# ethz-asl/laser_slam

Measured on AMD Instinct MI355X. Metric: scans_per_sec, higher is better.
Workload: dtype f32

## Files before the change

laser_slam_amd/csrc/lsgpu_icp.hip:

```cpp
#include <cstring>
#include <cmath>
#include <cstdio>
#include <cstdlib>
#include <string>
#include <vector>
#include <chrono>
#include <system_error>
#include <thread>
#include <utility>

#include <dlfcn.h>

#include <hip/hip_runtime.h>
#include <rccl/rccl.h>

#include "../../include/lsgpu_icp.h"
#include "lsgpu_grid.hip.h"
#include "lsgpu_tuning.h"
#include "lsgpu_policy.h"
#include "lsgpu_knn.hip.h"
#include "lsgpu_knn_k.hip.h"
#include "lsgpu_snf.hip.h"
#include "lsgpu_max_density.hip.h"
#include "lsgpu_cone.hip.h"
// ... 1683 lines not shown
    const bool fresh = h->ssn_bounds_ws.cap == 0;
    HIPC(h->ssn_bounds_ws.reserve(8 + 6 * kSsnBoundsBlocks));
    if (fresh) HIPC(hipMemsetAsync(h->ssn_bounds_ws.p, 0, 8 * sizeof(uint32_t), h->stream));
    hipLaunchKernelGGL(k_ssn_bounds_root, dim3(std::min(nblk(n), kSsnBoundsBlocks)), dim3(256), 0, h->stream, src, (int)n, h->ssn_bounds_ws.p,
                       h->ssn_bb.p, h->ssn_seg_a.p);
  }
  SsnSeg* cur = h->ssn_seg_a.p;
  SsnSeg* nxt = h->ssn_seg_b.p;
  const uint32_t* idx = nullptr;
  const int* root_axis = nullptr;
  int glevels = 0;
  const int root_auto = n >= 200ll * 8192 ? 8192 : n >= 200ll * 4096 ? 4096 : 2048;
  const int root_max = tuning().ssn_root ? tuning().ssn_root : root_auto;
  int root_levels = 0;
  while ((8 << root_levels) < root_max) ++root_levels;
  {
    int64_t c = n;
    while (glevels < levels && !(c <= root_max && levels - glevels <= root_levels)) { c -= c / 2; ++glevels; }
  }
  const bool select_levels = !force_sort_levels && !tuning().ssn_sort_levels && glevels > 0;
  const uint32_t* root_sig = nullptr;
  if (select_levels) {
    if (h->gs_plan_n != n || h->gs_plan_levels != glevels) {
      std::vector<uint32_t> sizes{(uint32_t)n}, next;
      h->gs_lvl_first.clear(); h->gs_lvl_blocks.clear();
      uint32_t rows = 0, segs = 0;
      for (int L = 0; L < glevels; ++L) {
        uint32_t fb = 0;
        next.clear();
        for (uint32_t c : sizes) {
          fb += (c + kGsTile - 1u) / kGsTile;
          next.push_back(c - c / 2u); next.push_back(c / 2u);
        }
        h->gs_lvl_first.push_back(rows); h->gs_lvl_blocks.push_back(fb);
        rows += fb; segs += (uint32_t)sizes.size();
        sizes.swap(next);
      }
      HIPC(h->gs_tab.reserve(rows)); HIPC(h->gs_sblk.reserve(segs));
      if (glevels <= kGsPlanLevels && ((size_t)1 << (glevels - 1)) <= kGsPlanSegs) {
        GsPlanArgs pa{};
        for (int L = 0; L < glevels; ++L) pa.first[L] = h->gs_lvl_first[L];
        hipLaunchKernelGGL(k_gs_plan, dim3(glevels), dim3(1024), 0, h->stream, (uint32_t)n, pa, h->gs_tab.p, h->gs_sblk.p);
        HIPC(hipGetLastError());
      } else {
        std::vector<GsBlock> tab;
        std::vector<GsSegBlocks> sblk;
        std::vector<std::pair<uint32_t, uint32_t>> segsz{{0u, (uint32_t)n}};
        for (int L = 0; L < glevels; ++L) {
          uint32_t fb = 0;
          std::vector<std::pair<uint32_t, uint32_t>> nx;
          for (uint32_t sidx = 0; sidx < segsz.size(); ++sidx) {
            const uint32_t st = segsz[sidx].first, c = segsz[sidx].second;
            const uint32_t nb = (c + kGsTile - 1u) / kGsTile;
            sblk.push_back(GsSegBlocks{fb, nb, st, c});
            for (uint32_t k = 0; k < nb; ++k)
              tab.push_back(GsBlock{st + k * kGsTile, std::min(kGsTile, c - k * kGsTile), sidx, st, c, fb, nb, 0u});
            fb += nb;
            const uint32_t left = c - c / 2u;
            nx.push_back({st, left}); nx.push_back({st + left, c - left});
          }
          segsz.swap(nx);
        }
        HIPC(hipMemcpyAsync(h->gs_tab.p, tab.data(), tab.size() * sizeof(GsBlock), hipMemcpyHostToDevice, h->stream));
        HIPC(hipMemcpyAsync(h->gs_sblk.p, sblk.data(), sblk.size() * sizeof(GsSegBlocks), hipMemcpyHostToDevice, h->stream));
        HIPC(hipStreamSynchronize(h->stream));
      }
      h->gs_plan_n = n; h->gs_plan_levels = glevels;
    }
    const size_t nseg_g = (size_t)1 << glevels;
    int cap = 1;
    for (uint32_t v : h->gs_lvl_blocks) cap = std::max(cap, (int)v);
    for (auto& bf : h->gs_e) HIPC(bf.reserve(n));
    for (auto& bf : h->gs_k) HIPC(bf.reserve(n));
    HIPC(h->gs_hist.reserve(4 * 256 * (nseg_g + 1))); HIPC(h->gs_median.reserve(nseg_g)); HIPC(h->gs_cand_n.reserve(2 * nseg_g + 2));
    const size_t cand_room = std::max<size_t>(nseg_g / 2, 1) * kGsCandRoom;
    HIPC(h->gs_cand.reserve(cand_room)); HIPC(h->gs_cand_blk.reserve(cand_room));
    HIPC(h->gs_cl.reserve((size_t)2 * cap)); HIPC(h->gs_err.reserve(8)); HIPC(h->gs_rng.reserve(2 * nseg_g + 2));
    HIPC(h->ssn_axis_a.reserve(nseg_g)); HIPC(h->ssn_axis_b.reserve(nseg_g));
    if (!h->h_gs_err) HIPC(hipHostMalloc((void**)&h->h_gs_err, 64, hipHostMallocDefault));
    uint32_t* cand_n[2] = {h->gs_cand_n.p, h->gs_cand_n.p + nseg_g + 1};
    uint32_t* sig_cur = reinterpret_cast<uint32_t*>(h->ssn_axis_a.p);
    uint32_t* sig_nxt = reinterpret_cast<uint32_t*>(h->ssn_axis_b.p);
    GsSet in, out;
    in.e = h->gs_e[0].p; out.e = h->gs_e[1].p;
    for (int d = 0; d < 3; ++d) { in.k[d] = h->gs_k[d].p; out.k[d] = h->gs_k[3 + d].p; }
    uint2* rng_cur = h->gs_rng.p;
    uint2* rng_nxt = h->gs_rng.p + nseg_g + 1;
    uint32_t* gh1[2] = {h->gs_hist.p, h->gs_hist.p + 256 * (nseg_g + 1)};
    uint32_t* gh2[2] = {h->gs_hist.p + 2 * 256 * (nseg_g + 1), h->gs_hist.p + 3 * 256 * (nseg_g + 1)};
    hipLaunchKernelGGL(k_gs_init, dim3(nblk(n)), dim3(256), 0, h->stream, src, (int)n, in, out.e, (const SsnSeg*)cur, (const uint32_t*)h->ssn_bb.p, rng_cur,
                       gh1[0], gh2[0], cand_n[0], sig_cur, h->gs_err.p);
    for (int L = 0; L < glevels; ++L) {
      const int ns = 1 << L, nb = (int)h->gs_lvl_blocks[L], par = L & 1;
      const GsBlock* tab = h->gs_tab.p + h->gs_lvl_first[L];
      const GsSegBlocks* sblk = h->gs_sblk.p + (ns - 1);
      hipLaunchKernelGGL(k_gs_hist<1>, dim3(nb), dim3(256), 0, h->stream, tab, cur, (const uint2*)rng_cur, in, gh1[par], gh2[par], h->gs_err.p);
      hipLaunchKernelGGL(k_gs_hist<2>, dim3(nb), dim3(256), 0, h->stream, tab, cur, (const uint2*)rng_cur, in, gh1[par], gh2[par], h->gs_err.p);
      const uint32_t lvl_cap = (uint32_t)std::min<size_t>(cand_room / (size_t)ns, (size_t)1 << 22);
      hipLaunchKernelGGL(k_gs_collect, dim3(nb), dim3(256), 0, h->stream, tab, cur, (const uint2*)rng_cur, (const uint32_t*)sig_cur, in,
                         (const uint32_t*)gh1[par], (const uint32_t*)gh2[par], cand_n[par], h->gs_cand.p, h->gs_cand_blk.p, lvl_cap, h->gs_cl.p);
      hipLaunchKernelGGL(k_gs_select, dim3(ns), dim3(L < 3 ? 1024 : 256), 0, h->stream, sblk, src, cur, (const uint32_t*)sig_cur, gh1[par], gh2[par],
                         gh1[par ^ 1], gh2[par ^ 1], cand_n[par], (const GsMedian*)h->gs_cand.p, (const uint32_t*)h->gs_cand_blk.p, lvl_cap, h->gs_cl.p,
                         h->gs_cl.p + cap, h->gs_median.p, nxt, sig_nxt, cand_n[par ^ 1], rng_nxt, h->gs_err.p);
      hipLaunchKernelGGL(k_gs_part, dim3(nb), dim3(kGsPartThreads), 0, h->stream, tab, cur, (const uint32_t*)sig_cur, in, out,
                         (const GsMedian*)h->gs_median.p, (const uint32_t*)(h->gs_cl.p + cap), (const SsnSeg*)nxt, rng_nxt, h->gs_err.p);
      std::swap(in, out);
      std::swap(cur, nxt);
      std::swap(sig_cur, sig_nxt);
      std::swap(rng_cur, rng_nxt);
    }
    idx = in.e;
    root_sig = sig_cur;
    HIPC(hipGetLastError());
  } else if (glevels > 0) {
    const size_t nseg_g = (size_t)1 << glevels;
    const int cap = (int)(n / kSegTile + (int64_t)(nseg_g / 2) + 2);
    HIPC(h->lane.scratch->vals_alt.reserve(n));
    HIPC(h->ssn_axis_a.reserve(nseg_g)); HIPC(h->ssn_axis_b.reserve(nseg_g)); HIPC(h->ssn_seg_fb.reserve(nseg_g));
    HIPC(h->ssn_blocktab.reserve((size_t)cap)); HIPC(h->lane.scratch->sort_hist.reserve((size_t)256 * cap + 256 + 4));
    uint32_t* keyA = reinterpret_cast<uint32_t*>(h->lane.scratch->keys.p);
    uint32_t* keyB = keyA + n;
    uint32_t* valA = h->lane.scratch->vals.p;
    uint32_t* valB = h->lane.scratch->vals_alt.p;
    uint32_t* bh = h->lane.scratch->sort_hist.p;
    uint32_t* dtot = bh + (size_t)256 * cap;
    uint32_t* nblocks_dev = dtot + 256;
    int* ax_cur = h->ssn_axis_a.p;
    int* ax_nxt = h->ssn_axis_b.p;
    HIPC(hipMemsetAsync(ax_cur, 0xFF, sizeof(int), h->stream));
    for (int L = 0; L < glevels; ++L) {
      const int ns = 1 << L;
      const int grid = (int)std::min<int64_t>(cap, n / kSegTile + ns + 1);
      hipLaunchKernelGGL(k_ssn_plan, dim3(1), dim3(256), 0, h->stream, cur, ns, knn, ax_cur, h->ssn_seg_fb.p,
                         h->ssn_blocktab.p, nblocks_dev);
      hipLaunchKernelGGL(k_ssn_keys32, dim3(nblk(n)), dim3(256), 0, h->stream, src, (int)n, valA, h->ssn_seg_of.p, cur,
                         h->ssn_seg_fb.p, L == 0 ? 1 : 0, keyA);
      for (int pass = 0; pass < 4; ++pass) {
        const uint32_t* kin = (pass & 1) ? keyB : keyA; const uint32_t* vin = (pass & 1) ? valB : valA;
        uint32_t* kout = (pass & 1) ? keyA : keyB; uint32_t* vout = (pass & 1) ? valA : valB;
        hipLaunchKernelGGL(k_seg_hist<kSegItems>, dim3(grid), dim3(256), 0, h->stream, kin, h->ssn_blocktab.p, nblocks_dev, 8 * pass, bh, cap);
        hipLaunchKernelGGL(k_seg_scan, dim3(256), dim3(256), 0, h->stream, bh, cap, nblocks_dev, dtot);
        hipLaunchKernelGGL((k_seg_scatter<kSegItems>), dim3(grid), dim3(256), 0, h->stream, kin, vin, kout, vout,
                           h->ssn_blocktab.p, nblocks_dev, 8 * pass, bh, dtot, cap);
      }
      idx = valA;
      hipLaunchKernelGGL(k_ssn_split, dim3(nblk(ns)), dim3(256), 0, h->stream, src, idx, cur, ns, knn, nxt, (const int*)ax_cur, ax_nxt);
      hipLaunchKernelGGL(k_ssn_assign, dim3(nblk(n)), dim3(256), 0, h->stream, (int)n, cur, knn, h->ssn_seg_of.p, L == 0 ? 1 : 0);
      std::swap(cur, nxt);
      std::swap(ax_cur, ax_nxt);
    }
    root_axis = ax_cur;
    HIPC(hipGetLastError());
  }
  if (glevels < levels) {
    if (glevels == 0) {
      hipLaunchKernelGGL(k_ssn_keys, dim3(nblk(n)), dim3(256), 0, h->stream, src, (int)n, (const uint32_t*)nullptr,
                         (const uint32_t*)nullptr, cur, knn, h->lane.scratch->keys.p, h->lane.scratch->vals.p);
      idx = h->lane.scratch->vals.p;
    }
    uint32_t* idx_rw = const_cast<uint32_t*>(idx);
    if (root_max == 8192)
      hipLaunchKernelGGL(k_ssn_tree<8192>, dim3(1 << glevels), dim3(1024), 0, h->stream, src, idx_rw, cur, knn, levels - glevels, h->ssn_seg_of.p, nxt, root_axis, root_sig);
    else if (root_max == 4096)
      hipLaunchKernelGGL(k_ssn_tree<4096>, dim3(1 << glevels), dim3(512), 0, h->stream, src, idx_rw, cur, knn, levels - glevels, h->ssn_seg_of.p, nxt, root_axis, root_sig);
    else
      hipLaunchKernelGGL(k_ssn_tree<2048>, dim3(1 << glevels), dim3(256), 0, h->stream, src, idx_rw, cur, knn, levels - glevels, h->ssn_seg_of.p, nxt, root_axis, root_sig);
    std::swap(cur, nxt);
  }
  if (levels == 0) {
    hipLaunchKernelGGL(k_ssn_keys, dim3(nblk(n)), dim3(256), 0, h->stream, src, (int)n, (const uint32_t*)nullptr,
                       (const uint32_t*)nullptr, cur, knn, h->lane.scratch->keys.p, h->lane.scratch->vals.p);
    HIPC(hipMemsetAsync(h->ssn_seg_of.p, 0, (size_t)n * 4, h->stream));
    idx = h->lane.scratch->vals.p;
  }
  hipLaunchKernelGGL(k_ssn_boxes, dim3((int)((nseg + 127) / 128)), dim3(128), 0, h->stream, src, idx, cur, (int)nseg,
                     h->ssn_box_normal.p, h->ssn_box_pts.p);
  HIPC(hipGetLastError());
  int rc = scan_u32(h, h->ssn_box_pts.p, h->ssn_box_base.p, nseg);
  if (rc) return rc;
  rc = ahead->ready(first_draw + (size_t)n);
  if (rc) return rc;
  hipLaunchKernelGGL(k_ssn_select, dim3(nblk(n)), dim3(256), 0, h->stream, (int)n, idx, h->ssn_seg_of.p, cur,
                     h->ssn_box_pts.p, h->ssn_box_base.p, h->ssn_draws.p + first_draw, ratio, h->ssn_keep.p);
  rc = scan_u32(h, h->ssn_keep.p, h->ssn_out_pos.p, (size_t)n, false,  true);
  if (rc == LSGPU_OK) {
    hipLaunchKernelGGL(k_ssn_emit, dim3(nblk(n)), dim3(256), 0, h->stream, src, (int)n,
                       h->ssn_box_normal.p, h->ssn_keep.p, h->ssn_out_pos.p, out_xyz1, out_nrm);
  }
  uint32_t n_draws = 0, kept = 0;
  if (rc == LSGPU_OK)
    rc = scan_totals(h, h->ssn_box_pts.p, h->ssn_box_base.p, nseg, h->ssn_keep.p, h->ssn_out_pos.p, (size_t)n, &n_draws, &kept,
                     select_levels ? h->gs_err.p : nullptr, h->h_gs_err, 8 * sizeof(uint32_t),  true);
  if (rc) return rc;
  if (select_levels && *h->h_gs_err) {
    if (getenv("LSGPU_GS_DEBUG")) fprintf(stderr, "lsgpu: sort-free levels gave up (n %lld): code %u seg %u a %u b %u | part %u seg %u dst %u\n", (long long)n,
                                          h->h_gs_err[1], h->h_gs_err[2], h->h_gs_err[3], h->h_gs_err[4], h->h_gs_err[5], h->h_gs_err[6], h->h_gs_err[7]);
    ++h->ssn_sort_fallbacks;
    return ssn_device(h, src, n, knn, ratio, seed, out_xyz1, out_nrm, n_out, ahead, true);
  }
  ahead->used = first_draw + (size_t)n_draws;
  HIPC(hipGetLastError());
  *n_out = kept;
  return LSGPU_OK;
}

static int random_sampling_device(lsgpu_icp* h, const float4* src, int64_t n, float prob, int64_t seed,
                                  float4* out_xyz1, int64_t* n_out, DrawAhead* ahead = nullptr, bool defer_wait = false) {
  *n_out = 0;
  HIPC(h->ssn_keep.reserve(n));
  HIPC(h->ssn_out_pos.reserve(n));
  DrawAhead own;
  int rc = LSGPU_OK;
  if (!ahead) {
    rc = own.begin(h, seed, (size_t)n);
    if (rc) return rc;
    ahead = &own;
  }
  const size_t first_draw = ahead->used;
  ahead->used = first_draw + (size_t)n;
  rc = ahead->ready();
  if (rc) return rc;
  hipLaunchKernelGGL(k_draw_select, dim3(nblk(n)), dim3(256), 0, h->lane.stream, (int)n, h->ssn_draws.p + first_draw, prob, h->ssn_keep.p);
  rc = compact_kept_enqueue(h, src, n, out_xyz1);
  if (rc || defer_wait) return rc;
  return compact_kept_wait(h, n_out);
}

static CutSectionDev cut_section_of(const lsgpu_chain_cuts& c, int side, bool rs) {
  CutSectionDev d;
  std::memset(&d, 0, sizeof(d));
  const lsgpu_point_filter* m = side == 0 ? c.reading : c.reference;
  d.n = std::max(0, std::min(side == 0 ? c.n_reading : c.n_reference, kCutMax));
  d.n_pre = side == 0 && rs ? std::max(0, std::min(c.reading_sampling_at, d.n)) : d.n;
  for (int k = 0; k < d.n; ++k) {
    d.m[k].type = m[k].type; d.m[k].dim = m[k].dim; d.m[k].flag = m[k].flag;
    for (int i = 0; i < 6; ++i) d.m[k].v[i] = m[k].v[i];
  }
  return d;
}
static int cut_section_enqueue(lsgpu_icp* h, const CutSectionDev& cs, bool rs, float prob, const float* draws, const float4* src,
                               int64_t n, float4* dst) {
  const int nb = nblk(n);
  const size_t row = ((size_t)nb + 3) & ~(size_t)3;
  HIPC(h->cut_blk.reserve(4 * row));
  uint32_t *cnt_a = h->cut_blk.p, *off_a = cnt_a + row, *cnt_b = off_a + row, *off_b = cnt_b + row;
  hipStream_t st = h->lane.stream;
  hipLaunchKernelGGL((k_cut_pass<0, false>), dim3(nb), dim3(256), 0, st, src, (int)n, cs, (const float*)nullptr, 0.f,
                     (const uint32_t*)nullptr, (const uint32_t*)nullptr, cnt_a, (float4*)nullptr);
  int rc = scan_u32(h, cnt_a, off_a, (size_t)nb);
  if (rc) return rc;
  if (!rs) {
    hipLaunchKernelGGL((k_cut_pass<2, false>), dim3(nb), dim3(256), 0, st, src, (int)n, cs, (const float*)nullptr, 0.f,
                       (const uint32_t*)nullptr, (const uint32_t*)off_a, (uint32_t*)nullptr, dst);
    HIPC(hipGetLastError());
    return scan_totals_enqueue(h, nullptr, nullptr, 0, cnt_a, off_a, (size_t)nb);
  }
  hipLaunchKernelGGL((k_cut_pass<1, true>), dim3(nb), dim3(256), 0, st, src, (int)n, cs, draws, prob, (const uint32_t*)off_a,
                     (const uint32_t*)nullptr, cnt_b, (float4*)nullptr);
  rc = scan_u32(h, cnt_b, off_b, (size_t)nb);
  if (rc) return rc;
  hipLaunchKernelGGL((k_cut_pass<2, true>), dim3(nb), dim3(256), 0, st, src, (int)n, cs, draws, prob, (const uint32_t*)off_a,
                     (const uint32_t*)off_b, (uint32_t*)nullptr, dst);
  HIPC(hipGetLastError());
  return scan_totals_enqueue(h, cnt_a, off_a, (size_t)nb, cnt_b, off_b, (size_t)nb);
}
static int cut_section_wait(lsgpu_icp* h, bool rs, int64_t* pre, int64_t* kept) {
  uint32_t a = 0, b = 0;
  const int rc = scan_totals_wait(h, &a, &b);
  if (rc) return rc;
  *kept = b;
  *pre = rs ? a : b;
  return LSGPU_OK;
}

template <int K, bool DENS>
static void launch_snf_(lsgpu_icp* h, const SnfArgs& a) {
  hipLaunchKernelGGL((k_snf_tile<K, DENS>), dim3((unsigned)((a.n + 63) / 64)), dim3(64), 0, h->stream, a);
  hipLaunchKernelGGL((k_snf_fallback<K, DENS>), dim3((unsigned)std::min((a.n + 63) / 64, 4096)), dim3(64), 0, h->stream, a);
}
template <int K>
static void launch_snf(lsgpu_icp* h, const SnfArgs& a) {
  if (a.dens) launch_snf_<K, true>(h, a); else launch_snf_<K, false>(h, a);
}
static int snf_device(lsgpu_icp* h, int knn, int* ids, float* d2, float* dens = nullptr) {
  const int64_t n = h->nr;
  if (knn < kSnfMinKnn || knn > kSnfMaxKnn || n < knn) {
    h->err = "SurfaceNormalDataPointsFilter: knn must be in [3, 32] and the cloud must hold at least knn points";
    return LSGPU_BAD_ARG;
  }
  HIPC(h->snf_strag.reserve(n)); HIPC(h->snf_count.reserve(1));
  HIPC(hipMemsetAsync(h->snf_count.p, 0, sizeof(uint32_t), h->stream));
  SnfArgs a;
  a.n = (int)n; a.knn = knn; a.g = h->grid; a.pts = h->pts.p; a.inv = h->ref_inv.p; a.chunks = h->chunks.p;
  a.nrm = h->nrm.p; a.ids = ids; a.d2 = ids ? d2 : nullptr;
  a.strag = h->snf_strag.p; a.strag_count = h->snf_count.p; a.r_cap = kSnfRCap; a.dens = dens;
  if (knn <= 4) launch_snf<4>(h, a);
  else if (knn <= 8) launch_snf<8>(h, a);
  else if (knn <= 16) launch_snf<16>(h, a);
  else launch_snf<32>(h, a);
  HIPC(hipGetLastError());
  return LSGPU_OK;
}

static int max_density_enqueue(lsgpu_icp* h, const float4* src, int64_t n, const float* dens, float max_density,
                               const float* draws, bool normals, float4* out_pts, float* out_nrm) {
  const int nb = nblk(n);
  const size_t row = ((size_t)nb + 3) & ~(size_t)3;
  HIPC(h->md_blk.reserve(4 * row)); HIPC(h->md_stat.reserve(1));
  uint32_t *cnt_a = h->md_blk.p, *off_a = cnt_a + row, *cnt_b = off_a + row, *off_b = cnt_b + row;
  hipStream_t st = h->lane.stream;
  HIPC(hipMemsetAsync(h->md_stat.p, 0, sizeof(MdStat), st));
  HIPC(hipMemsetAsync(&h->md_stat.p->lo, 0xFF, sizeof(uint32_t), st));
  const uint32_t* inv = h->ref_inv.p;
  const float4* nrm = normals ? h->nrm.p : nullptr;
  hipLaunchKernelGGL((k_md_pass<0>), dim3(nb), dim3(256), 0, st, src, dens, (int)n, max_density, (const float*)nullptr, h->md_stat.p,
                     (const uint32_t*)nullptr, (const uint32_t*)nullptr, cnt_a, inv, nrm, (float4*)nullptr, (float*)nullptr);
  int rc = scan_u32(h, cnt_a, off_a, (size_t)nb);
  if (rc) return rc;
  hipLaunchKernelGGL((k_md_pass<1>), dim3(nb), dim3(256), 0, st, src, dens, (int)n, max_density, draws, h->md_stat.p,
                     (const uint32_t*)off_a, (const uint32_t*)nullptr, cnt_b, inv, nrm, (float4*)nullptr, (float*)nullptr);
  rc = scan_u32(h, cnt_b, off_b, (size_t)nb);
  if (rc) return rc;
  hipLaunchKernelGGL((k_md_pass<2>), dim3(nb), dim3(256), 0, st, src, dens, (int)n, max_density, draws, h->md_stat.p,
                     (const uint32_t*)off_a, (const uint32_t*)off_b, (uint32_t*)nullptr, inv, nrm, out_pts, out_nrm);
  HIPC(hipGetLastError());
  return scan_totals_enqueue(h, cnt_a, off_a, (size_t)nb, cnt_b, off_b, (size_t)nb);
}
static int max_density_wait(lsgpu_icp* h, int64_t* n_dense, int64_t* kept) {
  uint32_t a = 0, b = 0;
// ... 1486 lines not shown
```

laser_slam_amd/csrc/lsgpu_ssn_tree.hip.h:

```cpp
#pragma once
#include "lsgpu_ssn.hip.h"

namespace lsgpu {

struct alignas(8) TreeSeg {
  uint16_t start, count;
  uint8_t cut;
  uint8_t ord;
  uint16_t pad;
};
struct alignas(8) TreeBox { float lo[3], hi[3]; };

template <int B>
struct SsnTreeLds {
  static constexpr int T = B / 8;
  static constexpr int W = T / 64;
  static constexpr int S = B / 8;
  static constexpr int SP = B / 16;
  uint16_t rank[3][B];
  uint16_t list[3][B];
  union {
    struct { uint32_t key[B]; uint32_t cnt[W][256]; } pre;
    struct { uint16_t cur_pos[B]; uint16_t sof[B]; TreeBox box[SP]; uint32_t segbase[S]; } tree;
  } u;
  TreeSeg seg[S];
  uint32_t wsum[W];
  uint32_t wtot[4];
  uint32_t kmin[3], kmax[3];
};

#ifdef LSGPU_KNN_STATS
__device__ unsigned long long g_tree_dbg[64];
#define LSGPU_TREE_T(n) do { if (blockIdx.x == 0 && threadIdx.x == 0) g_tree_dbg[n] = (unsigned long long)clock64(); } while (0)
#else
#define LSGPU_TREE_T(n) do { } while (0)
#endif

#define LSGPU_TREE_SYNC() __syncthreads()

__device__ __forceinline__ uint32_t tree_lane_prev(uint32_t v) { return (uint32_t)__builtin_amdgcn_update_dpp(0, (int)v, 0x138, 0xF, 0xF, false); }
__device__ __forceinline__ uint32_t tree_lane_next(uint32_t v) { return (uint32_t)__builtin_amdgcn_update_dpp(0, (int)v, 0x130, 0xF, 0xF, false); }
__device__ __forceinline__ uint32_t tree_wave_scan(uint32_t v, int lane) {
  v = row_scan_incl_u32(v);
  const uint32_t t0 = rl_u(v, 15), t1 = rl_u(v, 31), t2 = rl_u(v, 47);
  return v + (lane >= 16 ? t0 : 0u) + (lane >= 32 ? t1 : 0u) + (lane >= 48 ? t2 : 0u);
}

template <int B>
__global__ __launch_bounds__(B / 8) void k_ssn_tree(const float4* __restrict__ p, uint32_t* __restrict__ idx,
                                                    const SsnSeg* __restrict__ segs, int knn, int rem,
                                                    uint32_t* __restrict__ seg_of, SsnSeg* __restrict__ segs_out,
                                                    const int* __restrict__ root_axis ,
                                                    const uint32_t* __restrict__ root_sig ) {
  using Lds = SsnTreeLds<B>;
  constexpr int T = Lds::T, W = Lds::W;
  __shared__ Lds L;
  const int tid = threadIdx.x, lane = tid & 63, w = tid >> 6;
  const SsnSeg root = segs[blockIdx.x];
  const int cnt = (int)root.count;
  const unsigned long long lt = (1ull << lane) - 1ull;
  const int sorted_axis = root_axis ? root_axis[blockIdx.x] : -1;

  LSGPU_TREE_T(0);
  uint32_t kx[8], ky[8], kz[8];
  if (tid < 3) { L.kmin[tid] = 0xFFFFFFFFu; L.kmax[tid] = 0u; }
  {
    uint32_t mn[3] = {0xFFFFFFFFu, 0xFFFFFFFFu, 0xFFFFFFFFu}, mx[3] = {0u, 0u, 0u};
#pragma unroll
    for (int it = 0; it < 8; ++it) {
      const int e = w * 512 + it * 64 + lane;
      kx[it] = ky[it] = kz[it] = 0u;
      if (e < cnt) {
        const float4 v = p[idx[root.start + e]];
        kx[it] = float_order_key(v.x); ky[it] = float_order_key(v.y); kz[it] = float_order_key(v.z);
        mn[0] = min(mn[0], kx[it]); mx[0] = max(mx[0], kx[it]);
        mn[1] = min(mn[1], ky[it]); mx[1] = max(mx[1], ky[it]);
        mn[2] = min(mn[2], kz[it]); mx[2] = max(mx[2], kz[it]);
      }
    }
    __syncthreads();
#pragma unroll
    for (int d = 0; d < 3; ++d) {
      const uint32_t a = ~wave_max_u32(~mn[d]), b = wave_max_u32(mx[d]);
      if (lane == 0) { atomicMin(&L.kmin[d], a); atomicMax(&L.kmax[d], b); }
    }
    __syncthreads();
  }

  LSGPU_TREE_T(1);
#pragma unroll
  for (int d = 0; d < 3; ++d) {
    const uint32_t kmin = L.kmin[d];
    const uint32_t range = cnt > 0 ? L.kmax[d] - kmin : 0u;
    const int bits = range ? 32 - __clz((int)range) : 0;
    const int P = d == sorted_axis ? 0 : (bits + 7) >> 3;
#pragma unroll
    for (int it = 0; it < 8; ++it) {
      const int e = w * 512 + it * 64 + lane;
      const uint32_t k = d == 0 ? kx[it] : d == 1 ? ky[it] : kz[it];
      if (e < cnt) L.u.pre.key[e] = k - kmin;
    }
    __syncthreads();
    for (int j = 0; j < P; ++j) {
      uint16_t* dst = ((P - 1 - j) & 1) ? L.rank[d] : L.list[d];
      const uint16_t* src = ((P - 1 - j) & 1) ? L.list[d] : L.rank[d];
      const int shift = 8 * j;
#pragma unroll
      for (int q = 0; q < 4; ++q) (&L.u.pre.cnt[0][0])[tid + q * T] = 0u;
      __syncthreads();
      uint32_t es[8], dg[8], rk[8];
#pragma unroll
      for (int it = 0; it < 8; ++it) {
        const int i = w * 512 + it * 64 + lane;
        const bool valid = i < cnt;
        const uint32_t e = valid ? (j == 0 ? (uint32_t)i : (uint32_t)src[i]) : 0u;
        const uint32_t dgt = valid ? (L.u.pre.key[e] >> shift) & 255u : 0u;
        es[it] = e; dg[it] = dgt;
        unsigned long long peers = __ballot(valid);
#pragma unroll
        for (int b = 0; b < 8; ++b) {
          const bool bit = (dgt >> b) & 1u;
          const unsigned long long m = __ballot(bit);
          peers &= bit ? m : ~m;
        }
        const int leader = valid ? __ffsll((long long)peers) - 1 : lane;
        uint32_t old = 0u;
        if (valid && lane == leader) {
          old = L.u.pre.cnt[w][dgt];
          L.u.pre.cnt[w][dgt] = old + (uint32_t)__popcll(peers);
        }
        old = (uint32_t)__shfl((int)old, leader, 64);
        rk[it] = old + (uint32_t)__popcll(peers & lt);
        __builtin_amdgcn_wave_barrier();
        asm volatile("" ::: "memory");
      }
      __syncthreads();
      uint32_t tot = 0u, incl = 0u;
      if (tid < 256) {
#pragma unroll
        for (int ww = 0; ww < W; ++ww) tot += L.u.pre.cnt[ww][tid];
        incl = wave_scan_incl_u32(tot, lane);
        if (lane == 63) L.wtot[w] = incl;
      }
      __syncthreads();
      if (tid < 256) {
        uint32_t run = incl - tot;
        for (int ww = 0; ww < w; ++ww) run += L.wtot[ww];
#pragma unroll
        for (int ww = 0; ww < W; ++ww) {
          const uint32_t c = L.u.pre.cnt[ww][tid];
          L.u.pre.cnt[ww][tid] = run;
          run += c;
        }
      }
      __syncthreads();
#pragma unroll
      for (int it = 0; it < 8; ++it) {
        const int i = w * 512 + it * 64 + lane;
        if (i < cnt) dst[L.u.pre.cnt[w][dg[it]] + rk[it]] = (uint16_t)es[it];
      }
      __syncthreads();
    }
    if (P == 0) {
#pragma unroll
      for (int it = 0; it < 8; ++it) {
        const int i = w * 512 + it * 64 + lane;
        if (i < cnt) L.list[d][i] = (uint16_t)i;
      }
      __syncthreads();
    }
    LSGPU_TREE_T(2 + 2 * d);
#ifdef LSGPU_KNN_STATS
    if (blockIdx.x == 0 && tid == 0) g_tree_dbg[40 + d] = (unsigned long long)P;
#endif
    {
      uint32_t e[8], r[8];
      uint32_t carry = 0u;
#pragma unroll
      for (int k = 0; k < 8; ++k) {
        const int i = w * 512 + k * 64 + lane;
        e[k] = 0u;
        uint32_t kk = 0u;
        if (i < cnt) { e[k] = L.list[d][i]; kk = L.u.pre.key[e[k]]; }
        uint32_t pk = tree_lane_prev(kk);
        if (lane == 0 && i > 0 && i < cnt) pk = L.u.pre.key[L.list[d][i - 1]];
        const uint32_t f = (i < cnt && i > 0 && kk != pk) ? 1u : 0u;
        const uint32_t incl = tree_wave_scan(f, lane);
        r[k] = carry + incl;
        carry += rl_u(incl, 63);
      }
      if (lane == 0) L.wsum[w] = carry;
      __syncthreads();
      uint32_t before = 0u;
      for (int ww = 0; ww < w; ++ww) before += L.wsum[ww];
#pragma unroll
      for (int k = 0; k < 8; ++k)
        if (w * 512 + k * 64 + lane < cnt) L.rank[d][e[k]] = (uint16_t)(before + r[k]);
      __syncthreads();
    }
    LSGPU_TREE_T(3 + 2 * d);
  }

#pragma unroll
  for (int k = 0; k < 8; ++k) {
    const int i = w * 512 + k * 64 + lane;
    L.u.tree.cur_pos[i] = (uint16_t)i;
    L.u.tree.sof[i] = 0;
  }
  if (tid == 0) {
    TreeSeg r0;
    r0.start = 0; r0.count = (uint16_t)cnt; r0.cut = (uint8_t)ssn_cut_axis(root); r0.ord = 0xFF; r0.pad = 0;
    L.seg[0] = r0;
    TreeBox b0;
#pragma unroll
    for (int d = 0; d < 3; ++d) { b0.lo[d] = root.lo[d]; b0.hi[d] = root.hi[d]; }
    L.u.tree.box[0] = b0;
  }
  __syncthreads();
  const uint32_t rsig = root_sig ? root_sig[blockIdx.x] : 0xFFFFFFFFu;
  const uint32_t ro1 = rsig & 0xFFu, ro2 = (rsig >> 8) & 0xFFu, ro3 = (rsig >> 16) & 0xFFu;
  if (ro1 < 3u) {
    uint16_t* la = L.list[ro1];
    const uint16_t* ra = L.rank[ro1];
    const uint16_t* r2 = L.rank[ro2 < 3u ? ro2 : 0u];
    const uint16_t* r3 = L.rank[ro3 < 3u ? ro3 : 0u];
    uint32_t ek[8], np[8];
#pragma unroll
    for (int k = 0; k < 8; ++k) {
      const int i = w * 512 + k * 64 + lane;
      ek[k] = 0u; np[k] = (uint32_t)i;
      const bool act = i < cnt;
      if (act) ek[k] = la[i];
      const uint32_t r = act ? (uint32_t)ra[ek[k]] : 0xFFFFFFFFu;
      uint32_t rp = tree_lane_prev(r), rn = tree_lane_next(r);
      if (lane == 0 && act && i > 0) rp = ra[la[i - 1]];
      if (lane == 63 && act && i + 1 < cnt) rn = ra[la[i + 1]];
      if (act && ((i > 0 && rp == r) || (i + 1 < cnt && rn == r))) {
        int lo = i, hi = i + 1;
        while (lo > 0 && ra[la[lo - 1]] == r) --lo;
        while (hi < cnt && ra[la[hi]] == r) ++hi;
        const uint32_t e = ek[k];
        const uint32_t e2 = ro2 < 3u ? (uint32_t)r2[e] : 0u, e3 = ro3 < 3u ? (uint32_t)r3[e] : 0u;
        uint32_t c = 0u;
        for (int j = lo; j < hi; ++j) {
          const uint32_t f = la[j];
          const uint32_t f2 = ro2 < 3u ? (uint32_t)r2[f] : 0u, f3 = ro3 < 3u ? (uint32_t)r3[f] : 0u;
          const bool less = f2 != e2 ? f2 < e2 : f3 != e3 ? f3 < e3 : f < e;
          c += less ? 1u : 0u;
        }
        np[k] = (uint32_t)lo + c;
      }
    }
    __syncthreads();
#pragma unroll
    for (int k = 0; k < 8; ++k) {
      const int i = w * 512 + k * 64 + lane;
      if (i < cnt) { la[np[k]] = (uint16_t)ek[k]; L.u.tree.cur_pos[ek[k]] = (uint16_t)np[k]; }
    }
    if (tid == 0) L.seg[0].ord = (uint8_t)ro1;
    __syncthreads();
  }
  const uint32_t base_seg = (uint32_t)blockIdx.x << rem;
  for (int l = 0; l < rem; ++l) {
    const int ns = 1 << l;
    const bool last = l + 1 == rem;
    LSGPU_TREE_T(8 + l);
    uint32_t sk[8];
    TreeSeg sg[8];
#pragma unroll
    for (int k = 0; k < 8; ++k) {
      const int i = w * 512 + k * 64 + lane;
      sk[k] = L.u.tree.sof[i];
      sg[k] = L.seg[i < cnt ? sk[k] : 0u];
    }
    uint32_t ek[8], np[8];
    bool upd[8], fix[8];
#pragma unroll
    for (int k = 0; k < 8; ++k) {
      const int i = w * 512 + k * 64 + lane;
      const bool active = i < cnt && (int)sg[k].count > knn;
      const int a = sg[k].cut;
      upd[k] = active && sg[k].ord != a;
      fix[k] = upd[k] && sg[k].ord != 0xFF;
      ek[k] = 0u; np[k] = (uint32_t)i;
      const uint16_t* la = L.list[a];
      const uint16_t* ra = L.rank[a];
      if (upd[k]) ek[k] = la[i];
      if (__ballot(fix[k])) {
        const uint32_t r = fix[k] ? (uint32_t)ra[ek[k]] : 0xFFFFFFFFu;
        const int s0 = sg[k].start, s1 = s0 + sg[k].count;
        uint32_t rp = tree_lane_prev(r), rn = tree_lane_next(r);
        if (lane == 0 && fix[k] && i > s0) rp = ra[la[i - 1]];
        if (lane == 63 && fix[k] && i + 1 < s1) rn = ra[la[i + 1]];
        const bool tie = fix[k] && ((i > s0 && rp == r) || (i + 1 < s1 && rn == r));
        if (tie) {
          int lo = i, hi = i + 1;
          while (lo > s0 && ra[la[lo - 1]] == r) --lo;
          while (hi < s1 && ra[la[hi]] == r) ++hi;
          const uint32_t cp = L.u.tree.cur_pos[ek[k]];
          uint32_t c = 0u;
          for (int j = lo; j < hi; ++j) c += L.u.tree.cur_pos[la[j]] < cp ? 1u : 0u;
          np[k] = (uint32_t)lo + c;
        }
      }
    }
    LSGPU_TREE_SYNC();
#pragma unroll
    for (int k = 0; k < 8; ++k) {
      if (fix[k]) L.list[sg[k].cut][np[k]] = (uint16_t)ek[k];
      if (upd[k]) L.u.tree.cur_pos[ek[k]] = (uint16_t)np[k];
    }
    LSGPU_TREE_SYNC();
    TreeSeg ps;
    TreeBox pb;
    uint32_t gi = 0u;
    ps.start = 0; ps.count = 0; ps.cut = 0; ps.ord = 0xFF; ps.pad = 0;
    if (tid < ns) {
      ps = L.seg[tid];
      pb = L.u.tree.box[tid];
      if ((int)ps.count > knn) {
        const uint32_t left = (uint32_t)ps.count - (uint32_t)ps.count / 2u;
        gi = idx[root.start + L.list[ps.cut][ps.start + left]];
      }
    }
    uint32_t e1[8], e2[8], xk[8], vk[8];
    uint32_t carry = 0u;
#pragma unroll
    for (int k = 0; k < 8; ++k) {
      const int i = w * 512 + k * 64 + lane;
      const bool active = i < cnt && (int)sg[k].count > knn;
      uint32_t v = 0u;
      e1[k] = e2[k] = 0u;
      if (active) {
        const int a = sg[k].cut;
        const int d1 = a == 2 ? 0 : a + 1, d2 = a == 0 ? 2 : a - 1;
        const uint32_t left = (uint32_t)sg[k].count - (uint32_t)sg[k].count / 2u;
        e1[k] = L.list[d1][i]; e2[k] = L.list[d2][i];
        const uint32_t f1 = ((uint32_t)L.u.tree.cur_pos[e1[k]] - sg[k].start) >= left ? 1u : 0u;
        const uint32_t f2 = ((uint32_t)L.u.tree.cur_pos[e2[k]] - sg[k].start) >= left ? 1u : 0u;
        v = f1 | (f2 << 16);
      }
      vk[k] = v;
      const uint32_t incl = tree_wave_scan(v, lane);
      xk[k] = carry + incl - v;
      carry += rl_u(incl, 63);
    }
    if (lane == 0) L.wsum[w] = carry;
    LSGPU_TREE_SYNC();
    uint32_t before = 0u;
    for (int ww = 0; ww < w; ++ww) before += L.wsum[ww];
#pragma unroll
    for (int k = 0; k < 8; ++k) {
      xk[k] += before;
      const int i = w * 512 + k * 64 + lane;
      if (i < cnt && (int)sg[k].count > knn && i == (int)sg[k].start) L.u.tree.segbase[sk[k]] = xk[k];
    }
    LSGPU_TREE_SYNC();
#pragma unroll
    for (int k = 0; k < 8; ++k) {
      const int i = w * 512 + k * 64 + lane;
      uint32_t nsof = 2u * sk[k];
      if (i < cnt && (int)sg[k].count > knn) {
        const int a = sg[k].cut;
        const int d1 = a == 2 ? 0 : a + 1, d2 = a == 0 ? 2 : a - 1;
        const uint32_t left = (uint32_t)sg[k].count - (uint32_t)sg[k].count / 2u;
        const uint32_t rel = xk[k] - L.u.tree.segbase[sk[k]];
        const uint32_t r1 = rel & 0xFFFFu, r2 = rel >> 16;
        const uint32_t off = (uint32_t)i - sg[k].start;
        const uint32_t f1 = vk[k] & 1u, f2 = vk[k] >> 16;
        const uint32_t p1 = f1 ? sg[k].start + left + r1 : sg[k].start + (off - r1);
        const uint32_t p2 = f2 ? sg[k].start + left + r2 : sg[k].start + (off - r2);
        L.list[d1][p1] = (uint16_t)e1[k];
        L.list[d2][p2] = (uint16_t)e2[k];
        nsof += off >= left ? 1u : 0u;
      }
      L.u.tree.sof[i] = (uint16_t)nsof;
    }
    if (tid < ns) {
      TreeSeg ca = ps, cb = ps;
      TreeBox ba = pb, bb = pb;
      if ((int)ps.count > knn) {
        const int cut = ps.cut;
        const uint32_t right = (uint32_t)ps.count / 2u, left = (uint32_t)ps.count - right;
        const float cutval = coord_of(p[gi], cut);
        SsnSeg ta, tb;
#pragma unroll
        for (int d = 0; d < 3; ++d) {
          ba.hi[d] = d == cut ? cutval : ba.hi[d];
          bb.lo[d] = d == cut ? cutval : bb.lo[d];
          ta.lo[d] = ba.lo[d]; ta.hi[d] = ba.hi[d]; tb.lo[d] = bb.lo[d]; tb.hi[d] = bb.hi[d];
        }
        ca.count = (uint16_t)left; ca.cut = (uint8_t)ssn_cut_axis(ta); ca.ord = (uint8_t)cut;
        cb.start = (uint16_t)(ps.start + left); cb.count = (uint16_t)right; cb.cut = (uint8_t)ssn_cut_axis(tb); cb.ord = (uint8_t)cut;
      } else {
        cb.start = (uint16_t)(ps.start + ps.count); cb.count = 0;
      }
      L.seg[2 * tid] = ca;
      L.seg[2 * tid + 1] = cb;
      if (!last) {
        L.u.tree.box[2 * tid] = ba;
        L.u.tree.box[2 * tid + 1] = bb;
      } else {
        SsnSeg oa, ob;
        oa.start = root.start + ca.start; oa.count = ca.count;
        ob.start = root.start + cb.start; ob.count = cb.count;
#pragma unroll
        for (int d = 0; d < 3; ++d) { oa.lo[d] = ba.lo[d]; oa.hi[d] = ba.hi[d]; ob.lo[d] = bb.lo[d]; ob.hi[d] = bb.hi[d]; }
        segs_out[base_seg + 2u * (uint32_t)tid] = oa;
        segs_out[base_seg + 2u * (uint32_t)tid + 1u] = ob;
      }
    }
    LSGPU_TREE_SYNC();
  }

  LSGPU_TREE_T(30);
  uint32_t g[8], so[8];
#pragma unroll
  for (int k = 0; k < 8; ++k) {
    const int i = w * 512 + k * 64 + lane;
    g[k] = 0u; so[k] = 0u;
    if (i < cnt) {
      so[k] = L.u.tree.sof[i];
      const TreeSeg leaf = L.seg[so[k]];
      const uint32_t e = leaf.ord == 0xFF ? (uint32_t)i : (uint32_t)L.list[leaf.ord][i];
      g[k] = idx[root.start + e];
    }
  }
  __syncthreads();
#pragma unroll
  for (int k = 0; k < 8; ++k) {
    const int i = w * 512 + k * 64 + lane;
    if (i < cnt) {
      idx[root.start + i] = g[k];
      seg_of[root.start + i] = base_seg + so[k];
    }
  }
  LSGPU_TREE_T(31);
}

}
```

laser_slam_amd/csrc/lsgpu_tuning.h:

```cpp

#pragma once
#include <cstdio>
#include <cstdlib>
#include <cstring>

extern char** environ;

namespace lsgpu {

struct Tuning {
  int query_order = -1;
  float q_elev = 0.f, q_sect = 0.f;
  float gap = 0.002f;
  int chunk_budget = 512, chunk_budget_wide = 1024;
  int wide_iters = 3;
  float route_r = 0.02f;
  int route_chunks = 1024;
  int route_heavy_max = 1024;
  int route_dense = 512;
  bool predict_select = true, commit_select = true, comm_commit = true, seed_cap = true;
  int sel_amb_cap = 256;
  bool two_pass_select = true;
  bool short_last_group = true;
  bool fused_select = true;
  bool lazy_need = true;
  bool lane_split = true;
  bool lookahead = true;
  bool index_rest = true;
  bool side_stream = true;
  int front_guess = 2048;
  int sort_items = 0;
  bool ssn_sort_levels = false;
  int ssn_root = 0;
  int ne_blocks = 256;
  bool split_update = false;
  double comm_timeout_ms = 30000.0;
  int knn_dbg = 0;
  bool cone = true;
  bool cone_probe = true;
  int cone_rows = 128, cone_cols = 8192, cone_from = 2;
  float cone_max_occupancy = 7.0f;
  float cone_heavy_steps = 1024.f;
  float cone_heavy_share = 0.07f;
};

namespace tuning_detail {
inline bool flag(const char* name) { return getenv(name) != nullptr; }
inline double number(const char* name, double def, double lo, double hi) {
  const char* e = getenv(name);
  if (!e) return def;
  char* end = nullptr;
  const double v = strtod(e, &end);
  if (end == e || *end != '\0' || !(v >= lo && v <= hi)) {
    fprintf(stderr, "liblsgpu_icp: %s=%s is not a number in [%g, %g]; using the default %g\n", name, e, lo, hi, def);
    return def;
  }
  return v;
}
inline Tuning read() {
  Tuning t;
  t.query_order = (int)number("LSGPU_QUERY_ORDER", -1, -1, 1);
  t.q_elev = (float)number("LSGPU_Q_ELEV", 0, 0, 45);
  t.q_sect = (float)number("LSGPU_Q_SECT", 0, 0, 45);
  t.gap = (float)number("LSGPU_GAP", 0.002, 0, 1);
  t.chunk_budget = (int)number("LSGPU_BUDGET", 512, 1, 1 << 20);
  t.chunk_budget_wide = (int)number("LSGPU_BUDGET_WIDE", 1024, 1, 1 << 20);
  t.wide_iters = (int)number("LSGPU_WIDE_ITERS", 3, 0, 1 << 20);
  t.route_r = (float)number("LSGPU_ROUTE_R", 0.02, 1e-6, 1e6);
  t.route_chunks = (int)number("LSGPU_ROUTE_CHUNKS", 1024, 1, 1 << 30);
  t.route_heavy_max = (int)number("LSGPU_ROUTE_HEAVY_MAX", 1024, -1, 1 << 30);
  t.route_dense = (int)number("LSGPU_ROUTE_DENSE", 512, 1, 1 << 30);
  t.split_update = flag("LSGPU_SPLIT_UPDATE");
  t.predict_select = !flag("LSGPU_NO_PREDICT") && !t.split_update;
  t.commit_select = !flag("LSGPU_NO_COMMIT");
  t.fused_select = !flag("LSGPU_NO_FUSED_SELECT");
  t.short_last_group = !flag("LSGPU_FULL_GROUPS");
  t.two_pass_select = !flag("LSGPU_THREE_PASS_SELECT");
  t.sel_amb_cap = (int)number("LSGPU_SEL_AMB_CAP", 256, 0, 256);
  t.comm_commit = !flag("LSGPU_NO_COMM_COMMIT");
  t.seed_cap = !flag("LSGPU_NO_SEED_CAP");
  t.lazy_need = !flag("LSGPU_NO_LAZY");
  t.lane_split = !flag("LSGPU_NO_SPLIT");
  t.side_stream = !flag("LSGPU_NO_SIDE_STREAM");
  t.lookahead = !flag("LSGPU_NO_LOOKAHEAD");
  t.index_rest = !flag("LSGPU_NO_INDEX_REST");
  t.front_guess = (int)number("LSGPU_FRONT_GUESS", 2048, 0, 8192);
  t.sort_items = (int)number("LSGPU_SORT_ITEMS", 0, 0, 16);
  if (t.sort_items != 0 && t.sort_items != 4 && t.sort_items != 8 && t.sort_items != 16) {
    fprintf(stderr, "liblsgpu_icp: LSGPU_SORT_ITEMS must be 4, 8 or 16; choosing by size\n");
    t.sort_items = 0;
  }
  t.ssn_sort_levels = flag("LSGPU_SSN_SORT_LEVELS");
  t.ssn_root = (int)number("LSGPU_SSN_ROOT", 0, 0, 8192);
  if (t.ssn_root != 0 && t.ssn_root != 2048 && t.ssn_root != 4096 && t.ssn_root != 8192) {
    fprintf(stderr, "liblsgpu_icp: LSGPU_SSN_ROOT must be 2048, 4096 or 8192; choosing by size\n");
    t.ssn_root = 0;
  }
  t.ne_blocks = (int)number("LSGPU_NE_BLOCKS", 256, 64, 2048);
  t.comm_timeout_ms = number("LSGPU_COMM_TIMEOUT_MS", 30000, 1, 1e9);
  t.knn_dbg = (int)number("LSGPU_KNN_DBG", 0, 0, 1 << 20);
  t.cone = !flag("LSGPU_NO_CONE");
  t.cone_probe = !flag("LSGPU_NO_CONE_PROBE");
  t.cone_from = (int)number("LSGPU_CONE_FROM", 2, 1, 1 << 20);
  t.cone_max_occupancy = (float)number("LSGPU_CONE_MAX_OCC", 7.0, 0.0, 1e9);
  t.cone_heavy_steps = (float)number("LSGPU_CONE_HEAVY_STEPS", 1024.0, 0.0, 1e9);
  t.cone_heavy_share = (float)number("LSGPU_CONE_HEAVY_SHARE", 0.07, 0.0, 2.0);
  t.cone_rows = (int)number("LSGPU_CONE_ROWS", 128, 8, 1024);
  t.cone_cols = (int)number("LSGPU_CONE_COLS", 8192, 64, 65536) & ~3;
  static const char* known[] = {"LSGPU_QUERY_ORDER", "LSGPU_Q_ELEV", "LSGPU_Q_SECT", "LSGPU_GAP", "LSGPU_BUDGET", "LSGPU_BUDGET_WIDE", "LSGPU_WIDE_ITERS",
                                "LSGPU_ROUTE_R", "LSGPU_ROUTE_CHUNKS", "LSGPU_ROUTE_HEAVY_MAX", "LSGPU_ROUTE_DENSE", "LSGPU_SPLIT_UPDATE", "LSGPU_NO_PREDICT", "LSGPU_NO_COMMIT",
                                "LSGPU_NO_COMM_COMMIT", "LSGPU_NO_SEED_CAP", "LSGPU_NO_LAZY", "LSGPU_NO_SPLIT", "LSGPU_NO_SIDE_STREAM", "LSGPU_NO_LOOKAHEAD", "LSGPU_NO_INDEX_REST", "LSGPU_CELLS_SPLIT", "LSGPU_NO_FUSED_SELECT", "LSGPU_FULL_GROUPS", "LSGPU_THREE_PASS_SELECT", "LSGPU_SEL_AMB_CAP", "LSGPU_FRONT_GUESS",
                                "LSGPU_SORT_ITEMS", "LSGPU_SSN_ROOT", "LSGPU_SSN_SORT_LEVELS",
                                "LSGPU_NE_BLOCKS", "LSGPU_COMM_TIMEOUT_MS", "LSGPU_KNN_DBG", "LSGPU_NO_CONE", "LSGPU_NO_CONE_PROBE", "LSGPU_CONE_ROWS", "LSGPU_CONE_COLS", "LSGPU_CONE_FROM", "LSGPU_CONE_MAX_OCC", "LSGPU_CONE_HEAVY_STEPS", "LSGPU_CONE_HEAVY_SHARE",
                                "LSGPU_SO", "LSGPU_STATS_SO", "LSGPU_BATCH_POOLS", "LSGPU_BATCH_UNIQ", "LSGPU_GS_DEBUG", "LSGPU_GOLDEN_DIR", "LSGPU_SEQ_PERTURB", "LSGPU_SEQ_POSES", "LSGPU_TEST_INPUT_FILTERS",
                                nullptr};
  for (char** e = environ; e && *e; ++e) {
    if (strncmp(*e, "LSGPU_", 6) != 0) continue;
    const char* eq = strchr(*e, '=');
    const size_t len = eq ? (size_t)(eq - *e) : strlen(*e);
    bool ok = false;
    for (const char** k = known; *k; ++k) ok = ok || (strlen(*k) == len && strncmp(*k, *e, len) == 0);
    if (!ok) fprintf(stderr, "liblsgpu_icp: unknown switch %.*s ignored (see csrc/lsgpu_tuning.h)\n", (int)len, *e);
  }
  return t;
}
}

inline const Tuning& tuning() {
  static const Tuning t = tuning_detail::read();
  return t;
}

}
```

Measured before the change: 249.1.

## Fuse leaf box-normal computation into SSN tree kernel using LDS-cached coordinates

Caches point coordinates in shared memory inside the k_ssn_tree kernel for root sizes up to 4096. The cached values serve two purposes: reading cut values without a gather from global memory, and computing per-leaf box normals and point counts at the end of the kernel. This removes the separate k_ssn_boxes launch and its global gathers. In exchange, LDS use grows by 12 bytes per point, which may lower occupancy, and the leaf normal work runs on one thread per leaf.

```diff
diff --git a/laser_slam_amd/csrc/lsgpu_icp.hip b/laser_slam_amd/csrc/lsgpu_icp.hip
--- a/laser_slam_amd/csrc/lsgpu_icp.hip
+++ b/laser_slam_amd/csrc/lsgpu_icp.hip
@@ -1859,6 +1859,7 @@
     root_axis = ax_cur;
     HIPC(hipGetLastError());
   }
+  bool tree_boxes = false;
   if (glevels < levels) {
     if (glevels == 0) {
       hipLaunchKernelGGL(k_ssn_keys, dim3(nblk(n)), dim3(256), 0, h->stream, src, (int)n, (const uint32_t*)nullptr,
@@ -1866,12 +1867,15 @@
       idx = h->lane.scratch->vals.p;
     }
     uint32_t* idx_rw = const_cast<uint32_t*>(idx);
+    tree_boxes = root_max <= 4096 && !tuning().ssn_split_boxes;
+    float* bn = tree_boxes ? h->ssn_box_normal.p : nullptr;
+    uint32_t* bp = tree_boxes ? h->ssn_box_pts.p : nullptr;
     if (root_max == 8192)
-      hipLaunchKernelGGL(k_ssn_tree<8192>, dim3(1 << glevels), dim3(1024), 0, h->stream, src, idx_rw, cur, knn, levels - glevels, h->ssn_seg_of.p, nxt, root_axis, root_sig);
+      hipLaunchKernelGGL(k_ssn_tree<8192>, dim3(1 << glevels), dim3(1024), 0, h->stream, src, idx_rw, cur, knn, levels - glevels, h->ssn_seg_of.p, nxt, root_axis, root_sig, bn, bp);
     else if (root_max == 4096)
-      hipLaunchKernelGGL(k_ssn_tree<4096>, dim3(1 << glevels), dim3(512), 0, h->stream, src, idx_rw, cur, knn, levels - glevels, h->ssn_seg_of.p, nxt, root_axis, root_sig);
+      hipLaunchKernelGGL(k_ssn_tree<4096>, dim3(1 << glevels), dim3(512), 0, h->stream, src, idx_rw, cur, knn, levels - glevels, h->ssn_seg_of.p, nxt, root_axis, root_sig, bn, bp);
     else
-      hipLaunchKernelGGL(k_ssn_tree<2048>, dim3(1 << glevels), dim3(256), 0, h->stream, src, idx_rw, cur, knn, levels - glevels, h->ssn_seg_of.p, nxt, root_axis, root_sig);
+      hipLaunchKernelGGL(k_ssn_tree<2048>, dim3(1 << glevels), dim3(256), 0, h->stream, src, idx_rw, cur, knn, levels - glevels, h->ssn_seg_of.p, nxt, root_axis, root_sig, bn, bp);
     std::swap(cur, nxt);
   }
   if (levels == 0) {
@@ -1880,8 +1884,9 @@
     HIPC(hipMemsetAsync(h->ssn_seg_of.p, 0, (size_t)n * 4, h->stream));
     idx = h->lane.scratch->vals.p;
   }
-  hipLaunchKernelGGL(k_ssn_boxes, dim3((int)((nseg + 127) / 128)), dim3(128), 0, h->stream, src, idx, cur, (int)nseg,
-                     h->ssn_box_normal.p, h->ssn_box_pts.p);
+  if (!tree_boxes)
+    hipLaunchKernelGGL(k_ssn_boxes, dim3((int)((nseg + 127) / 128)), dim3(128), 0, h->stream, src, idx, cur, (int)nseg,
+                       h->ssn_box_normal.p, h->ssn_box_pts.p);
   HIPC(hipGetLastError());
   int rc = scan_u32(h, h->ssn_box_pts.p, h->ssn_box_base.p, nseg);
   if (rc) return rc;
diff --git a/laser_slam_amd/csrc/lsgpu_ssn_tree.hip.h b/laser_slam_amd/csrc/lsgpu_ssn_tree.hip.h
--- a/laser_slam_amd/csrc/lsgpu_ssn_tree.hip.h
+++ b/laser_slam_amd/csrc/lsgpu_ssn_tree.hip.h
@@ -10,6 +10,8 @@
   uint16_t pad;
 };
 struct alignas(8) TreeBox { float lo[3], hi[3]; };
+
+template <int B> constexpr bool kSsnTreeCoords = B <= 4096;
 
 template <int B>
 struct SsnTreeLds {
@@ -27,6 +29,7 @@
   uint32_t wsum[W];
   uint32_t wtot[4];
   uint32_t kmin[3], kmax[3];
+  float xyz[3][kSsnTreeCoords<B> ? B : 1];
 };
 
 #ifdef LSGPU_KNN_STATS
@@ -51,9 +54,12 @@
                                                     const SsnSeg* __restrict__ segs, int knn, int rem,
                                                     uint32_t* __restrict__ seg_of, SsnSeg* __restrict__ segs_out,
                                                     const int* __restrict__ root_axis ,
-                                                    const uint32_t* __restrict__ root_sig ) {
+                                                    const uint32_t* __restrict__ root_sig ,
+                                                    float* __restrict__ box_normal ,
+                                                    uint32_t* __restrict__ box_pts) {
   using Lds = SsnTreeLds<B>;
   constexpr int T = Lds::T, W = Lds::W;
+  constexpr bool kCoords = kSsnTreeCoords<B>;
   __shared__ Lds L;
   const int tid = threadIdx.x, lane = tid & 63, w = tid >> 6;
   const SsnSeg root = segs[blockIdx.x];
@@ -73,6 +79,7 @@
       if (e < cnt) {
         const float4 v = p[idx[root.start + e]];
         kx[it] = float_order_key(v.x); ky[it] = float_order_key(v.y); kz[it] = float_order_key(v.z);
+        if constexpr (kCoords) { L.xyz[0][e] = v.x; L.xyz[1][e] = v.y; L.xyz[2][e] = v.z; }
         mn[0] = min(mn[0], kx[it]); mx[0] = max(mx[0], kx[it]);
         mn[1] = min(mn[1], ky[it]); mx[1] = max(mx[1], ky[it]);
         mn[2] = min(mn[2], kz[it]); mx[2] = max(mx[2], kz[it]);
@@ -314,13 +321,16 @@
     TreeSeg ps;
     TreeBox pb;
     uint32_t gi = 0u;
+    float cutval_lds = 0.f;
     ps.start = 0; ps.count = 0; ps.cut = 0; ps.ord = 0xFF; ps.pad = 0;
     if (tid < ns) {
       ps = L.seg[tid];
       pb = L.u.tree.box[tid];
       if ((int)ps.count > knn) {
         const uint32_t left = (uint32_t)ps.count - (uint32_t)ps.count / 2u;
-        gi = idx[root.start + L.list[ps.cut][ps.start + left]];
+        const uint32_t le = L.list[ps.cut][ps.start + left];
+        if constexpr (kCoords) cutval_lds = L.xyz[ps.cut][le];
+        else gi = idx[root.start + le];
       }
     }
     uint32_t e1[8], e2[8], xk[8], vk[8];
@@ -382,7 +392,8 @@
       if ((int)ps.count > knn) {
         const int cut = ps.cut;
         const uint32_t right = (uint32_t)ps.count / 2u, left = (uint32_t)ps.count - right;
-        const float cutval = coord_of(p[gi], cut);
+        float cutval;
+        if constexpr (kCoords) cutval = cutval_lds; else cutval = coord_of(p[gi], cut);
         SsnSeg ta, tb;
 #pragma unroll
         for (int d = 0; d < 3; ++d) {
@@ -436,6 +447,28 @@
     }
   }
   LSGPU_TREE_T(31);
+
+  if constexpr (kCoords) {
+    if (box_normal && tid < (1 << rem)) {
+      const TreeSeg leaf = L.seg[tid];
+      const uint16_t* ol = L.list[leaf.ord == 0xFF ? 0 : leaf.ord] + leaf.start;
+      const bool own = leaf.ord == 0xFF;
+      const int first = leaf.start;
+      const uint32_t s = base_seg + (uint32_t)tid;
+      uint32_t kept = 0u;
+      if (leaf.count > 0) {
+        float n[3];
+        if (boxnormal::box_normal((int)leaf.count, [&](int i, int d) { return L.xyz[d][own ? first + i : (int)ol[i]]; }, n)) {
+          kept = leaf.count;
+          box_normal[3 * (size_t)s + 0] = n[0];
+          box_normal[3 * (size_t)s + 1] = n[1];
+          box_normal[3 * (size_t)s + 2] = n[2];
+        }
+      }
+      box_pts[s] = kept;
+    }
+  }
+  LSGPU_TREE_T(32);
 }
 
 }
diff --git a/laser_slam_amd/csrc/lsgpu_tuning.h b/laser_slam_amd/csrc/lsgpu_tuning.h
--- a/laser_slam_amd/csrc/lsgpu_tuning.h
+++ b/laser_slam_amd/csrc/lsgpu_tuning.h
@@ -32,6 +32,7 @@
   int sort_items = 0;
   bool ssn_sort_levels = false;
   int ssn_root = 0;
+  bool ssn_split_boxes = false;
   int ne_blocks = 256;
   bool split_update = false;
   double comm_timeout_ms = 30000.0;
@@ -96,6 +97,7 @@
     fprintf(stderr, "liblsgpu_icp: LSGPU_SSN_ROOT must be 2048, 4096 or 8192; choosing by size\n");
     t.ssn_root = 0;
   }
+  t.ssn_split_boxes = flag("LSGPU_SSN_SPLIT_BOXES");
   t.ne_blocks = (int)number("LSGPU_NE_BLOCKS", 256, 64, 2048);
   t.comm_timeout_ms = number("LSGPU_COMM_TIMEOUT_MS", 30000, 1, 1e9);
   t.knn_dbg = (int)number("LSGPU_KNN_DBG", 0, 0, 1 << 20);
@@ -110,7 +112,7 @@
   static const char* known[] = {"LSGPU_QUERY_ORDER", "LSGPU_Q_ELEV", "LSGPU_Q_SECT", "LSGPU_GAP", "LSGPU_BUDGET", "LSGPU_BUDGET_WIDE", "LSGPU_WIDE_ITERS",
                                 "LSGPU_ROUTE_R", "LSGPU_ROUTE_CHUNKS", "LSGPU_ROUTE_HEAVY_MAX", "LSGPU_ROUTE_DENSE", "LSGPU_SPLIT_UPDATE", "LSGPU_NO_PREDICT", "LSGPU_NO_COMMIT",
                                 "LSGPU_NO_COMM_COMMIT", "LSGPU_NO_SEED_CAP", "LSGPU_NO_LAZY", "LSGPU_NO_SPLIT", "LSGPU_NO_SIDE_STREAM", "LSGPU_NO_LOOKAHEAD", "LSGPU_NO_INDEX_REST", "LSGPU_CELLS_SPLIT", "LSGPU_NO_FUSED_SELECT", "LSGPU_FULL_GROUPS", "LSGPU_THREE_PASS_SELECT", "LSGPU_SEL_AMB_CAP", "LSGPU_FRONT_GUESS",
-                                "LSGPU_SORT_ITEMS", "LSGPU_SSN_ROOT", "LSGPU_SSN_SORT_LEVELS",
+                                "LSGPU_SORT_ITEMS", "LSGPU_SSN_ROOT", "LSGPU_SSN_SORT_LEVELS", "LSGPU_SSN_SPLIT_BOXES",
                                 "LSGPU_NE_BLOCKS", "LSGPU_COMM_TIMEOUT_MS", "LSGPU_KNN_DBG", "LSGPU_NO_CONE", "LSGPU_NO_CONE_PROBE", "LSGPU_CONE_ROWS", "LSGPU_CONE_COLS", "LSGPU_CONE_FROM", "LSGPU_CONE_MAX_OCC", "LSGPU_CONE_HEAVY_STEPS", "LSGPU_CONE_HEAVY_SHARE",
                                 "LSGPU_SO", "LSGPU_STATS_SO", "LSGPU_BATCH_POOLS", "LSGPU_BATCH_UNIQ", "LSGPU_GS_DEBUG", "LSGPU_GOLDEN_DIR", "LSGPU_SEQ_PERTURB", "LSGPU_SEQ_POSES", "LSGPU_TEST_INPUT_FILTERS",
                                 nullptr};
```

Result: faster. 253.9 (median of 5 runs) (+1.9%).
